# FordyceLab/magnify

Hardware: AMD Instinct MI355X
Metric: megapixels/sec through flatfield+segment+ROI-reduce; markers/sec (higher is better)
Workload: dtype u16

## Files before the change

### include/magnify_hip.h

```cpp
#ifndef MAGNIFY_HIP_H
#define MAGNIFY_HIP_H

#include <stddef.h>
#include <stdint.h>

#ifdef __cplusplus
extern "C" {
#endif

#define MG_OK 0
#define MG_EINVAL (-1)
#define MG_ELAUNCH (-2)
#define MG_EIO (-3)

#define MG_U8 0
#define MG_U16 1
#define MG_F32 2
#define MG_F64 3

#define MG_NO_EDGE 100.0f
#define MG_SCORE_SKIPPED (-2.0f)


int mg_version(void);
// ... 32 lines not shown
                                    double dark, const void* d_dark, int dark_dtype,
                                    double flat, const void* d_flat, int flat_dtype,
                                    const double* d_max2, void* d_image, double* d_minmax, void* stream);

int mg_flatfield_apply_stitch_shift(const void* d_tiles, int dtype, int64_t n_planes, int n_tile_rows, int n_tile_cols,
                                    int ty, int tx, int overlap, int apply_flatfield, int planes_per_group,
                                    double dark, const void* d_dark, int dark_dtype,
                                    double flat, const void* d_flat, int flat_dtype,
                                    const double* d_max2, void* d_image, double* d_minmax,
                                    const int32_t* d_shift, int n_tables, int n_time, int blend, void* stream);


int64_t mg_seam_sums_scratch_bytes(int64_t n_planes, int n_tile_rows, int n_tile_cols, int ty, int tx, int overlap,
                                   int max_shift);
int mg_seam_sums(const void* d_planes, int dtype, int64_t n_planes, int n_tile_rows, int n_tile_cols, int ty, int tx,
                 int overlap, int max_shift, void* d_sums, void* d_fixed, void* d_scratch, int64_t scratch_bytes,
                 void* stream);


int mg_track_beads(const void* d_planes, int dtype, int n_t, int64_t plane_stride, int h, int w, int t_ref,
                   const int32_t* d_beads, int m, int half, int max_drift, int32_t* d_shift, double* d_score,
                   void* d_sums, void* d_fixed, void* stream);

int mg_track_beads_based(const void* d_planes, int dtype, int n_t, int64_t plane_stride, int h, int w, int t_ref,
                         const int32_t* d_beads, int m, int half, int max_drift, const int32_t* d_base,
                         int32_t* d_shift, double* d_score, void* d_sums, void* d_fixed, void* stream);

int mg_bin_planes(const void* d_planes, int dtype, int n_t, int64_t plane_stride, int h, int w, int bin,
                  float* d_out, void* stream);

int mg_plane_minmax(const void* d_src, int dtype, int n_planes, int64_t plane_stride, int h, int w,
                    int64_t row_stride, double* d_minmax, void* stream);


int mg_affine_bilinear(const void* d_src, void* d_dst, int dtype, int64_t n_planes, int h, int w,
                       const double* matrix, const double* offset, double* d_minmax, void* stream);

int64_t mg_shading_workspace_bytes(int n, int w);
int64_t mg_shading_offset(int n, int w, int field);
int mg_shading_downsample(const void* d_tiles, int dtype, int64_t n, int ty, int tx, int w, float* d_out, void* stream);
int mg_shading_prepare(void* d_ws, int n, int w, void* stream);
int mg_shading_dct2(void* d_ws, int n, int w, const double* d_in, double* d_out, int inverse, void* stream);
int mg_shading_alm_begin(void* d_ws, int n, int w, int get_darkfield, int max_iterations, double mu, double lam_f,
                         double lam_d, double tol, double norm_f, double b_up, void* stream);
int mg_shading_alm_iterate(void* d_ws, int n, int w, int k, int get_darkfield, void* stream);
int mg_shading_reweight(void* d_ws, int n, int w, double epsilon, void* stream);
int mg_shading_upsample(const double* d_flat_w, const double* d_dark_w, int w, int ty, int tx, double* d_partial,
                        float* d_flat, float* d_dark, void* stream);
int mg_shading_apply_stitch(const void* d_tiles, int dtype, int n_fields, int64_t planes_per_field, int n_tile_rows,
                            int n_tile_cols, int ty, int tx, int overlap, const float* d_flat, const float* d_dark,
                            void* d_image, double* d_minmax, void* stream);
int mg_shading_apply_stitch_blend(const void* d_tiles, int dtype, int n_fields, int64_t planes_per_field,
                                  int n_tile_rows, int n_tile_cols, int ty, int tx, int overlap, const float* d_flat,
                                  const float* d_dark, void* d_image, double* d_minmax, void* stream);

int mg_shading_apply_stitch_shift(const void* d_tiles, int dtype, int n_fields, int64_t planes_per_field,
                                  int n_tile_rows, int n_tile_cols, int ty, int tx, int overlap, const float* d_flat,
                                  const float* d_dark, void* d_image, double* d_minmax, const int32_t* d_shift,
                                  int n_tables, int n_time, int blend, void* stream);


int mg_to_uint8_blur(const void* d_src, int dtype, int n_planes, int64_t plane_stride, int h, int w,
                     int64_t row_stride, const double* d_minmax, uint8_t* d_blur, uint8_t* d_u8, void* stream);

int mg_scharr_hist(const uint8_t* d_blur, int n_planes, int h, int w, int mode, const uint32_t* d_base,
                   uint32_t* d_hist, uint32_t* d_scratch, int64_t scratch_words, void* stream);
int64_t mg_scharr_hist_scratch_words(int n_planes, int h, int w, int mode);

int mg_to_uint8_blur_hist(const void* d_src, int dtype, int n_planes, int64_t plane_stride, int h, int w,
                          int64_t row_stride, const double* d_minmax, uint8_t* d_blur, uint8_t* d_u8, uint32_t* d_hist,
                          uint32_t* d_scratch, int64_t scratch_words, void* stream);
int64_t mg_blur_hist_scratch_words(int n_planes, int h, int w);

int mg_edge_thresholds(const uint32_t* d_hist, int n_planes, const int64_t* ranks4, float gamma_low, float gamma_high,
                       int32_t* d_thresh, float* d_quantiles, int32_t* d_unresolved, int32_t* d_state,
                       uint32_t* d_win_base, void* stream);
int mg_edge_thresholds_window(const uint32_t* d_hist_win, int n_planes, int pass, float gamma_low, float gamma_high,
                              int32_t* d_state, uint32_t* d_win_base, int32_t* d_thresh, float* d_quantiles,
                              int32_t* d_unresolved, void* stream);


int mg_canny_nms(const uint8_t* d_blur, int n_planes, int h, int w, const int32_t* d_thresh, uint32_t* d_weak,
                 uint32_t* d_strong, uint32_t* d_class, int64_t words_per_plane, void* stream);

int mg_canny_hysteresis(const uint32_t* d_weak, uint32_t* d_strong, int64_t words_per_plane, int n_planes, int h,
                        int w, uint32_t* d_changed, const uint8_t* d_flags_in, uint8_t* d_flags_out, void* stream);
int mg_hysteresis_tiles(int h, int w, int* tiles_x, int* tiles_y);

int mg_unpack_bits(const uint32_t* d_bits, int64_t words_per_plane, int n_planes, int64_t n_bits, uint8_t* d_out,
                   void* stream);

int64_t mg_edge_grid_scan_words(int n_planes, int h, int w, int grid);
int mg_edge_grid(const uint32_t* d_edge_bits, int64_t words_per_plane, int n_planes, int h, int w, int grid,
                 int32_t* d_cell_counts, int32_t* d_cell_starts, int32_t* d_num_edges, int32_t* d_coords,
                 int64_t coord_cap, uint64_t* d_scan_state, int32_t* d_edge_totals, int phases, void* stream);

int mg_edge_angles(const uint8_t* d_blur, int n_planes, int h, int w, const int32_t* d_coords, int64_t coord_cap,
                   const int32_t* d_num_edges, float* d_angle, void* stream);


int mg_dedup_layout(int h, int w, int min_r, int max_r, int* n_tile_rows, int* n_tile_cols, int64_t* n_layers,
                    int64_t* bitmap_words);

int mg_candidate_circles(const int32_t* d_coords, int64_t coord_cap, const int32_t* d_cell_starts,
                         const int32_t* d_cell_counts, const int32_t* d_num_edges, int n_planes, int h, int w,
                         int grid, const uint64_t* d_seeds, int64_t num_iter, int min_r, int max_r,
                         uint32_t* d_bitmap, int64_t bitmap_words, float* d_raw, void* stream);

int mg_candidate_keys(const int32_t* d_coords, int64_t coord_cap, const int32_t* d_cell_starts,
                      const int32_t* d_cell_counts, const int32_t* d_num_edges, int n_planes, int h, int w, int grid,
                      const uint64_t* d_seeds, int64_t num_iter, int min_r, int max_r, uint32_t* d_keys, float* d_raw,
                      void* stream);

int mg_keys_to_circles(const uint32_t* d_keys, int64_t num_iter, const int32_t* d_cell_starts,
                       const int32_t* d_cell_counts, const int32_t* d_num_edges, int n_planes, int h, int w, int grid,
                       int min_r, int max_r, uint32_t* d_unique_keys, int64_t circle_cap, int32_t* d_tile_ranges,
                       int32_t* d_num_circles, int32_t* d_layer_starts, int counters_clear, void* stream);

int mg_bitmap_to_circles(uint32_t* d_bitmap, int64_t bitmap_words, int n_planes, int h, int w, int min_r,
                         int max_r, int32_t* d_layer_offsets, int32_t* d_circles, int64_t circle_cap,
                         int32_t* d_num_circles, void* stream);

int mg_score_circles(const float* d_angle, const uint32_t* d_edge_bits, const uint32_t* d_class_bits,
                     int64_t words_per_plane, int n_planes, int h, int w, int32_t* d_circles, int64_t circle_cap,
                     const int32_t* d_layer_offsets, const uint32_t* d_unique_keys, const int32_t* d_tile_ranges,
                     int min_r, int max_r, const int32_t* d_per_rc, const double* d_per_expected,
                     const int32_t* d_per_starts, int per_total, float min_roundness, int write_skipped,
                     int dedup_centres, float* d_scores, int32_t* d_alive, int32_t* d_num_alive, int32_t* d_max_rc,
                     int32_t* d_num_scored, void* stream);

int mg_score_keyed_supported(int min_r, int max_r);
int mg_score_pair_table(uint64_t* out_entries, int cap);
int mg_score_pairs(int r, int32_t* out_rc, int cap);
int mg_score_walk_reads(int r);
int mg_score_circles_keyed(const uint8_t* d_blur, const float* d_angle, const uint32_t* d_edge_bits,
                           const uint32_t* d_class_bits, int64_t words_per_plane, int n_planes, int h, int w,
                           int32_t* d_circles, int64_t circle_cap, const uint32_t* d_unique_keys,
                           const int32_t* d_layer_starts, int min_r, int max_r, const int32_t* d_per_rc,
                           const double* d_per_expected, const int32_t* d_per_starts, int per_total,
                           const uint64_t* d_pair_table, float min_roundness, int write_skipped, float* d_scores,
                           int32_t* d_alive, int32_t* d_num_alive, int32_t* d_max_rc, int32_t* d_num_scored,
                           int32_t* d_surv_list, int64_t surv_cap, int32_t* d_num_surv, int counters_clear,
                           void* stream);

int mg_nms_rounds(const int32_t* d_circles, int64_t circle_cap, const float* d_scores, const int32_t* d_alive,
                  const int32_t* d_num_alive, const int32_t* d_max_rc, int n_planes, int min_dist,
                  const int32_t* d_ring_rc, int ring_len, uint64_t* d_grid, int64_t grid_cap, uint8_t* d_state,
                  int32_t* d_undecided, int64_t undecided_stride, int n_rounds, int counters_clear,
                  const uint32_t* d_tie_keys, int64_t max_alive, const int32_t* d_skip, void* stream);

int mg_nms_same_centre(const int32_t* d_circles, int64_t circle_cap, const float* d_scores, const int32_t* d_alive,
                       const int32_t* d_num_alive, const int32_t* d_max_rc, int n_planes, int min_dist, uint64_t* d_grid,
                       int64_t grid_cap, uint8_t* d_state, const uint32_t* d_tie_keys, int64_t max_alive,
                       const int32_t* d_skip, void* stream);

int mg_nms_cleanup(const int32_t* d_circles, int64_t circle_cap, const float* d_scores, const int32_t* d_alive,
                   const int32_t* d_num_alive, const int32_t* d_max_rc, int n_planes, int min_dist,
                   const int32_t* d_ring_rc, int ring_len, uint64_t* d_grid, int64_t grid_cap, uint8_t* d_state,
                   int64_t max_alive, const int32_t* d_skip, void* stream);

int mg_nms_sparse(const int32_t* d_circles, int64_t circle_cap, const float* d_scores, const int32_t* d_alive,
                  const int32_t* d_num_alive, const int32_t* d_max_rc, int n_planes, int min_dist, const uint32_t* d_dbits,
                  uint8_t* d_state, const uint32_t* d_tie_keys, int32_t* d_done, void* stream);
int mg_nms_sparse_max_dist(void);

int mg_collect_circles(const int32_t* d_circles, int64_t circle_cap, const float* d_scores, const int32_t* d_alive,
// ... 137 lines not shown
```

### magnify_amd/csrc/mg_edges.hip

```cpp
#include <math.h>
#include <stdlib.h>

#include <algorithm>

#include "mg_common.h"

namespace {

constexpr int TW = 256;
constexpr int TH = 64;
constexpr int NT = 256;
constexpr int RPW = 16;
constexpr int LPAD = 16;
constexpr int LS = TW + 2 * LPAD;
constexpr int CHUNKS = LS / 16;

struct U8Scale {
  double mn, top, scale, offset;
  int passthrough;
};

__device__ __forceinline__ U8Scale make_scale(const double* d_minmax, int plane) {
  U8Scale s;
  s.passthrough = (d_minmax == nullptr);
// ... 74 lines not shown
        uint8_t v[16];
        decode_chunk<T>(raw[it], sc, v);
        store_chunk(tile, j, k, v);
      }
    }
    return;
  }
  const bool rows_ok = ((row_stride * sizeof(T)) & 15) == 0;
  uint4 raw[ITER][NLD];
  bool fast[ITER];
#pragma unroll
  for (int it = 0; it < ITER; ++it) {
    const int i = threadIdx.x + it * NT;
    fast[it] = false;
    if (i < TOTAL) {
      const auto [j, k] = row_col(i, CHUNKS);
      const int gy = mg_reflect101(ty0 - HALO + j, h), gx0 = tx0 - LPAD + 16 * k;
      const T* p = base + (int64_t)gy * row_stride + gx0;
      fast[it] = rows_ok && gx0 >= 0 && gx0 + 16 <= w && (reinterpret_cast<uintptr_t>(p) & 15) == 0;
      if (fast[it]) {
#pragma unroll
        for (int q = 0; q < NLD; ++q) raw[it][q] = reinterpret_cast<const uint4*>(p)[q];
      }
    }
  }
#pragma unroll
  for (int it = 0; it < ITER; ++it) {
    const int i = threadIdx.x + it * NT;
    if (i < TOTAL) {
      const auto [j, k] = row_col(i, CHUNKS);
      uint8_t v[16];
      if (fast[it]) {
        decode_chunk<T>(raw[it], sc, v);
      } else {
        const int gy = mg_reflect101(ty0 - HALO + j, h), gx0 = tx0 - LPAD + 16 * k;
        const T* rowp = base + (int64_t)gy * row_stride;
#pragma unroll
        for (int m = 0; m < 16; ++m) {
          const int c = 16 * k + m;
          const bool needed = c >= LPAD - HALO && c < LPAD + TW + HALO;
          v[m] = needed ? to_u8<T>(rowp[mg_reflect101(gx0 + m, w)], sc) : (uint8_t)0;
        }
      }
      store_chunk(tile, j, k, v);
    }
  }
}

struct Row12 {
  uint32_t d0, d1, d2;
  __device__ __forceinline__ int at(int off) const {
    const int b = off + 4;
    const uint32_t d = b < 4 ? d0 : (b < 8 ? d1 : d2);
    return (int)((d >> (8 * (b & 3))) & 0xFFu);
  }
};
__device__ __forceinline__ Row12 read_row(const uint8_t (*tile)[LS], int r, int c0) {
  const uint32_t* p = reinterpret_cast<const uint32_t*>(&tile[r][LPAD + c0 - 4]);
  return Row12{p[0], p[1], p[2]};
}

typedef short s2 __attribute__((ext_vector_type(2)));
typedef unsigned short u2 __attribute__((ext_vector_type(2)));

__device__ __forceinline__ u2 pair_01(uint32_t d) { return __builtin_bit_cast(u2, __builtin_amdgcn_perm(0u, d, 0x0C010C00u)); }
__device__ __forceinline__ u2 pair_12(uint32_t d) { return __builtin_bit_cast(u2, __builtin_amdgcn_perm(0u, d, 0x0C020C01u)); }
__device__ __forceinline__ u2 pair_23(uint32_t d) { return __builtin_bit_cast(u2, __builtin_amdgcn_perm(0u, d, 0x0C030C02u)); }
__device__ __forceinline__ u2 pair_across(uint32_t lo, uint32_t hi) {
  return __builtin_bit_cast(u2, __builtin_amdgcn_perm(hi, lo, 0x0C040C03u));
}
__device__ __forceinline__ uint32_t pack_bytes(uint32_t p01, uint32_t p23) { return __builtin_amdgcn_perm(p23, p01, 0x06040200u); }
__device__ __forceinline__ uint32_t zip_lo(s2 x, s2 y) {
  return __builtin_amdgcn_perm(__builtin_bit_cast(uint32_t, y), __builtin_bit_cast(uint32_t, x), 0x05040100u);
}
__device__ __forceinline__ uint32_t zip_hi(s2 x, s2 y) {
  return __builtin_amdgcn_perm(__builtin_bit_cast(uint32_t, y), __builtin_bit_cast(uint32_t, x), 0x07060302u);
}

__device__ __forceinline__ uint32_t wave_from_left(uint32_t v) {
  return (uint32_t)__builtin_amdgcn_update_dpp(0, (int)v, 0x138, 0xF, 0xF, false);
}
__device__ __forceinline__ uint32_t wave_from_right(uint32_t v) {
  return (uint32_t)__builtin_amdgcn_update_dpp(0, (int)v, 0x130, 0xF, 0xF, false);
}

template <int NP>
__device__ __forceinline__ void scharr_pairs(const u2 (&a)[NP], const u2 (&b)[NP], const u2 (&c)[NP],
                                             uint32_t (&xy)[2 * (NP - 1)]) {
  s2 S[NP], D[NP];
#pragma unroll
  for (int k = 0; k < NP; ++k) {
    S[k] = __builtin_bit_cast(s2, (u2)((a[k] + c[k]) * (unsigned short)3 + b[k] * (unsigned short)10));
    D[k] = __builtin_bit_cast(s2, c[k]) - __builtin_bit_cast(s2, a[k]);
  }
#pragma unroll
  for (int jp = 0; jp < NP - 1; ++jp) {
    const s2 dxp = S[jp + 1] - S[jp];
    const s2 mid = __builtin_bit_cast(s2, __builtin_amdgcn_alignbit(__builtin_bit_cast(uint32_t, D[jp + 1]),
                                                                     __builtin_bit_cast(uint32_t, D[jp]), 16));
    const s2 dyp = (D[jp] + D[jp + 1]) * (short)3 + mid * (short)10;
    xy[2 * jp] = zip_lo(dxp, dyp);
    xy[2 * jp + 1] = zip_hi(dxp, dyp);
  }
}
__device__ __forceinline__ int grad_sq(uint32_t xy) {
  return __builtin_amdgcn_sdot2(__builtin_bit_cast(s2, xy), __builtin_bit_cast(s2, xy), 0, false);
}

template <typename T>
__global__ __launch_bounds__(NT) void k_u8_blur(const T* __restrict__ src, int64_t plane_stride, int h, int w,
                                                int64_t row_stride, const double* __restrict__ d_minmax,
                                                uint8_t* __restrict__ d_blur, uint8_t* __restrict__ d_u8) {
  __shared__ __attribute__((aligned(16))) uint8_t tile[TH + 4][LS];
  const int plane = blockIdx.z;
  const int tx0 = blockIdx.x * TW, ty0 = blockIdx.y * TH;
  const U8Scale sc = make_scale(d_minmax, plane);
  load_tile<T, 2>(src + (int64_t)plane * plane_stride, row_stride, h, w, tx0, ty0, sc, tile);
  __syncthreads();
  const int lane = threadIdx.x & 63, wave = threadIdx.x >> 6;
  const int c0 = 4 * lane, gx = tx0 + c0;
  if (gx >= w) return;
  int hs[5][4];
  uint8_t* outp = d_blur + (int64_t)plane * h * w;
  uint8_t* rawp = d_u8 ? d_u8 + (int64_t)plane * h * w : nullptr;
  const bool full = (gx + 4 <= w) && ((w & 3) == 0);
#pragma unroll
  for (int jr = 0; jr < RPW + 4; ++jr) {
    const Row12 r = read_row(tile, wave * RPW + jr, c0);
#pragma unroll
    for (int k = 0; k < 4; ++k)
#pragma unroll
      for (int q = 0; q < 4; ++q) hs[k][q] = hs[k + 1][q];
#pragma unroll
    for (int q = 0; q < 4; ++q) hs[4][q] = r.at(q - 2) + 4 * r.at(q - 1) + 6 * r.at(q) + 4 * r.at(q + 1) + r.at(q + 2);
    if (rawp && jr >= 2 && jr < RPW + 2) {
      const int gy = ty0 + wave * RPW + jr - 2;
      if (gy < h) {
        if (full) *reinterpret_cast<uint32_t*>(rawp + (int64_t)gy * w + gx) = r.d1;
        else
          for (int q = 0; q < 4 && gx + q < w; ++q) rawp[(int64_t)gy * w + gx + q] = (uint8_t)r.at(q);
      }
    }
    if (jr >= 4) {
      const int gy = ty0 + wave * RPW + jr - 4;
      if (gy < h) {
        uint32_t packed = 0;
#pragma unroll
        for (int q = 0; q < 4; ++q) {
          const int v = hs[0][q] + 4 * hs[1][q] + 6 * hs[2][q] + 4 * hs[3][q] + hs[4][q];
          packed |= (uint32_t)((v + 128) >> 8) << (8 * q);
        }
        if (full) *reinterpret_cast<uint32_t*>(outp + (int64_t)gy * w + gx) = packed;
        else
          for (int q = 0; q < 4 && gx + q < w; ++q) outp[(int64_t)gy * w + gx + q] = (uint8_t)(packed >> (8 * q));
      }
    }
  }
}

constexpr int FINE = 8192;
constexpr int COARSE = 4096;
constexpr uint32_t MG_HIST_SKIP = 0xFFFFFFFFu;

constexpr int HIST_TILES = 3;

__device__ __forceinline__ void hist_add4_pairs(const u2 (&pa)[3], const u2 (&pb2)[3], const u2 (&pc)[3], int gx, int w,
// ... 387 lines not shown
  const int plane = blockIdx.x;
  int32_t* st = d_state + (int64_t)plane * TS_WORDS;
  const int n_win = st[TS_NWIN];
  if (pass >= n_win) return;
  int32_t coarse[4], resid[4];
#pragma unroll
  for (int k = 0; k < 4; ++k) coarse[k] = st[TS_COARSE + k], resid[k] = st[TS_RESID + k];
  const int cbin = nth_window(coarse, pass);
  const uint32_t* hist = d_hist_win + (int64_t)plane * FINE;
  constexpr int PER = FINE / NT;
  uint32_t mine_v[PER];
  long long mine = 0;
#pragma unroll
  for (int j = 0; j < PER; ++j) mine_v[j] = hist[threadIdx.x * PER + j], mine += mine_v[j];
  long long run = block_exscan_i64(mine, s_pre);
  if (threadIdx.x < 4) s_pos[threadIdx.x] = 0;
  __syncthreads();
#pragma unroll
  for (int j = 0; j < PER; ++j) {
    const long long nxt = run + mine_v[j];
#pragma unroll
    for (int k = 0; k < 4; ++k)
      if (coarse[k] == cbin && run <= (long long)resid[k] && (long long)resid[k] < nxt) s_pos[k] = threadIdx.x * PER + j;
    run = nxt;
  }
  __syncthreads();
  if (threadIdx.x == 0) {
    int32_t order[4];
#pragma unroll
    for (int k = 0; k < 4; ++k) {
      order[k] = st[TS_ORDER + k];
      if (coarse[k] == cbin) order[k] = (cbin << 13) + s_pos[k], st[TS_ORDER + k] = order[k];
    }
    const int left = n_win - 1 - pass;
    d_unresolved[plane] = left | (n_win << 8);
    d_win_base[plane] = left > 0 ? (uint32_t)nth_window(coarse, pass + 1) << 13 : MG_HIST_SKIP;
    if (left == 0) finish_thresholds(order, gamma_lo, gamma_hi, plane, d_thresh, d_quantiles);
  }
}

__device__ __forceinline__ uint32_t bits_at(const uint32_t* __restrict__ bits, int64_t bit0, int n) {
  const int64_t wi = bit0 >> 5;
  const int sh = (int)(bit0 & 31);
  uint64_t two = bits[wi];
  if (sh + n > 32) two |= (uint64_t)bits[wi + 1] << 32;
  const uint32_t v = (uint32_t)(two >> sh);
  return n >= 32 ? v : (v & ((1u << n) - 1u));
}
__device__ __forceinline__ uint32_t bits_at_nb(const uint32_t* __restrict__ bits, int64_t bit0, int n) {
  const int64_t wi = bit0 >> 5;
  const int sh = (int)(bit0 & 31);
  const uint64_t two = (uint64_t)bits[wi] | ((uint64_t)bits[wi + 1] << 32);
  const uint32_t v = (uint32_t)(two >> sh);
  return n >= 32 ? v : (v & ((1u << n) - 1u));
}
__device__ __forceinline__ void bits_or(uint32_t* __restrict__ bits, int64_t bit0, uint32_t v) {
  if (!v) return;
  const int64_t wi = bit0 >> 5;
  const int sh = (int)(bit0 & 31);
  atomicOr(&bits[wi], v << sh);
  if (sh && (v >> (32 - sh))) atomicOr(&bits[wi + 1], v >> (32 - sh));
}
__device__ __forceinline__ uint32_t row_word(const uint32_t* __restrict__ bits, int h, int w, int y, int x0) {
  if (y < 0 || y >= h) return 0u;
  const int lo = max(x0, 0), hi = min(x0 + 32, w);
  if (lo >= hi) return 0u;
  return bits_at(bits, (int64_t)y * w + lo, hi - lo) << (lo - x0);
}

__device__ __forceinline__ uint32_t shl1_or(uint32_t v, uint64_t mask) {
  uint32_t out;
  uint64_t carry_out;
  asm("v_addc_co_u32_e64 %0, %1, %2, %2, %3" : "=v"(out), "=s"(carry_out) : "v"(v), "s"(mask));
  return out;
}

__device__ __forceinline__ uint32_t or_reduce8(uint32_t v) {
  v |= (uint32_t)__builtin_amdgcn_update_dpp(0, (int)v, 0xB1, 0xF, 0xF, true);
  v |= (uint32_t)__builtin_amdgcn_update_dpp(0, (int)v, 0x4E, 0xF, 0xF, true);
  v |= (uint32_t)__builtin_amdgcn_update_dpp(0, (int)v, 0x141, 0xF, 0xF, true);
  return v;
}

__global__ __launch_bounds__(NT) void k_canny_nms(const uint8_t* __restrict__ d_blur, int h, int w,
                                                  const int32_t* __restrict__ d_thresh, int64_t words_per_plane,
                                                  uint32_t* __restrict__ d_weak, uint32_t* __restrict__ d_strong,
                                                  uint32_t* __restrict__ d_class) {
  __shared__ __attribute__((aligned(16))) uint8_t tile[TH + 4][LS];
  const int plane = blockIdx.z;
  const int tx0 = blockIdx.x * TW, ty0 = blockIdx.y * TH;
  load_tile<uint8_t, 2>(d_blur + (int64_t)plane * h * w, w, h, w, tx0, ty0, make_scale(nullptr, 0), tile);
  __syncthreads();
  const int low = d_thresh[2 * plane], high = d_thresh[2 * plane + 1];
  const int lane = threadIdx.x & 63, wave = threadIdx.x >> 6;
  const int c0 = 4 * lane, gx = tx0 + c0;
  uint32_t* weak = d_weak + plane * words_per_plane;
  uint32_t* strong = d_strong + plane * words_per_plane;
  uint32_t* cls0 = d_class ? d_class + (3 * plane) * words_per_plane : nullptr;
  uint32_t* cls1 = d_class ? d_class + (3 * plane + 1) * words_per_plane : nullptr;
  uint32_t* cls2 = d_class ? d_class + (3 * plane + 2) * words_per_plane : nullptr;
  constexpr int TG22 = 13573;
  const uint32_t in_row = gx + 4 <= w ? 0xFu : ((1u << max(w - gx, 0)) - 1u);
  struct Pairs4 {
    u2 p[4];
  };
  auto unpack = [](const Row12& r) {
    Pairs4 o;
    o.p[0] = pair_23(r.d0);
    o.p[1] = pair_01(r.d1);
    o.p[2] = pair_23(r.d1);
    o.p[3] = pair_01(r.d2);
    return o;
  };
  int mg[3][6];
  uint32_t cxy[2][4];
  Pairs4 ua = unpack(read_row(tile, wave * RPW, c0)), ub = unpack(read_row(tile, wave * RPW + 1, c0));
#pragma unroll
  for (int jr = 2; jr < RPW + 4; ++jr) {
    const Pairs4 uc = unpack(read_row(tile, wave * RPW + jr, c0));
    const int ym = ty0 - 2 + wave * RPW + jr - 1;
#pragma unroll
    for (int k = 0; k < 6; ++k) mg[0][k] = mg[1][k], mg[1][k] = mg[2][k];
#pragma unroll
    for (int q = 0; q < 4; ++q) cxy[0][q] = cxy[1][q];
    {
      uint32_t xy[6];
      scharr_pairs(ua.p, ub.p, uc.p, xy);
      const bool row_in = ym >= 0 && ym < h;
#pragma unroll
      for (int k = 0; k < 6; ++k) {
        const int x = gx + k - 1;
        const int m = grad_sq(xy[k]);
        mg[2][k] = (row_in && x >= 0 && x < w) ? m : 0;
        if (k >= 1 && k <= 4) cxy[1][k - 1] = xy[k];
      }
    }
    ua = ub;
    ub = uc;
    if (jr < 4) continue;
    const int yo = ym - 1;
    uint32_t wb = 0, sb = 0, cb0 = 0, cb1 = 0, cb2 = 0;
    if (yo < h) {
#pragma unroll
      for (int q = 3; q >= 0; --q) {
        const int m = mg[1][q + 1];
        const int xs = (int)(int16_t)(cxy[0][q] & 0xFFFFu), ys = (int)cxy[0][q] >> 16;
        const int x = abs(xs), ay = abs(ys), y = ay << 15;
        const int tg22x = x * TG22;
        const int tg67x = tg22x + (x << 16);
        const uint64_t horiz = __ballot(y < tg22x);
        const uint64_t vert = __ballot(y > tg67x) & ~horiz;
        const bool neg_b = (xs ^ ys) < 0;
        const uint64_t neg = __ballot(neg_b);
        const uint64_t ok_h = __ballot(m > mg[1][q]) & __ballot(m >= mg[1][q + 2]);
        const uint64_t ok_v = __ballot(m > mg[0][q + 1]) & __ballot(m >= mg[2][q + 1]);
        const uint64_t ok_d = __ballot(m > mg[0][q]) & __ballot(m > mg[2][q + 2]);
        const uint64_t ok_n = __ballot(m > mg[0][q + 2]) & __ballot(m > mg[2][q]);
        const uint64_t is_max = (horiz & ok_h) | (vert & ok_v) | (~(horiz | vert) & ((neg & ok_n) | (~neg & ok_d)));
        const uint64_t cand = is_max & __ballot(m > low) & __ballot(gx + q < w);
        wb = shl1_or(wb, cand);
        sb = shl1_or(sb, cand & __ballot(m > high));
        const bool le_b = ay <= x, ge_b = ay >= x;
        const uint64_t le = __ballot(le_b), ge = __ballot(ge_b);
        cb0 = shl1_or(cb0, (neg & le) | (~neg & ge));
        cb1 = shl1_or(cb1, neg);
        const bool lowq = neg_b ? le_b : !ge_b;
        const int sq = lowq ? x + ay : ay - x;
        const uint64_t upper = __ballot(sq * sq > 2 * x * x);
        cb2 = shl1_or(cb2, neg ^ upper);
      }
    }
    wb = or_reduce8(wb << (4 * (lane & 7)));
    sb = or_reduce8(sb << (4 * (lane & 7)));
    if (d_class) {
      cb0 = or_reduce8((cb0 & in_row) << (4 * (lane & 7)));
      cb1 = or_reduce8((cb1 & in_row) << (4 * (lane & 7)));
      cb2 = or_reduce8((cb2 & in_row) << (4 * (lane & 7)));
    }
    if ((lane & 7) == 0 && yo < h && gx < w) {
      const int64_t bit0 = (int64_t)yo * w + gx;
      if ((bit0 & 31) == 0 && gx + 32 <= w) {
        weak[bit0 >> 5] = wb;
        strong[bit0 >> 5] = sb;
        if (d_class) {
          cls0[bit0 >> 5] = cb0;
          cls1[bit0 >> 5] = cb1;
          cls2[bit0 >> 5] = cb2;
        }
      } else {
        bits_or(weak, bit0, wb);
        bits_or(strong, bit0, sb);
        if (d_class) {
          bits_or(cls0, bit0, cb0);
          bits_or(cls1, bit0, cb1);
          bits_or(cls2, bit0, cb2);
        }
      }
    }
  }
}

constexpr int HW = TW / 32;
constexpr int HTH = 256;

__device__ __forceinline__ bool hyst_interior(int r, int k) { return r >= 1 && r <= HTH && k >= 1 && k <= HW; }
__device__ __forceinline__ uint32_t lds_interior(const uint32_t (*a)[HW + 2], int r, int k) {
  return hyst_interior(r, k) ? a[r][k] : 0u;
}
template <typename At>
__device__ __forceinline__ uint32_t dilate3x3(At at, int r, int k) {
  uint32_t dil = 0;
#pragma unroll
  for (int dr = -1; dr <= 1; ++dr) {
    const uint32_t c = at(r + dr, k), l = at(r + dr, k - 1), rt = at(r + dr, k + 1);
    dil |= c | (c << 1) | (c >> 1) | (l >> 31) | (rt << 31);
  }
  return dil;
}

__global__ __launch_bounds__(NT) void k_hysteresis(const uint32_t* __restrict__ d_weak, uint32_t* __restrict__ d_strong,
                                                   int64_t words_per_plane, int h, int w,
                                                   uint32_t* __restrict__ d_changed,
                                                   const uint8_t* __restrict__ d_flags_in,
                                                   uint8_t* __restrict__ d_flags_out) {
  __shared__ uint32_t st[HTH + 2][HW + 2];
  __shared__ uint32_t wk[HTH + 2][HW + 2];
  __shared__ uint32_t s_mark;
  const int plane = blockIdx.z;
  const int tx0 = blockIdx.x * TW, ty0 = blockIdx.y * HTH;
  const int ntx = gridDim.x, nty = gridDim.y;
  if (d_flags_in && !d_flags_in[(int64_t)plane * ntx * nty + blockIdx.y * ntx + blockIdx.x]) return;
  const uint32_t* weak = d_weak + plane * words_per_plane;
  uint32_t* strong = d_strong + plane * words_per_plane;
  int pending = 0;
  if ((w & 31) == 0) {
    constexpr int TOTAL = (HTH + 2) * (HW + 2), ITER = (TOTAL + NT - 1) / NT;
    uint32_t sv[ITER], wv[ITER];
#pragma unroll
    for (int it = 0; it < ITER; ++it) {
      const int i = min((int)threadIdx.x + it * NT, TOTAL - 1);
      const auto [r, kk] = row_col(i, HW + 2);
      const int y = ty0 - 1 + r, x = tx0 - 32 + 32 * kk;
      const bool in = y >= 0 && y < h && x >= 0 && x < w;
      const int64_t wi = in ? ((int64_t)y * w + x) >> 5 : 0;
      sv[it] = strong[wi];
      wv[it] = weak[wi];
      if (!in) sv[it] = 0u, wv[it] = 0u;
    }
#pragma unroll
    for (int it = 0; it < ITER; ++it) {
      const int i = threadIdx.x + it * NT;
      if (i < TOTAL) {
        const auto [r, kk] = row_col(i, HW + 2);
        st[r][kk] = sv[it];
        wk[r][kk] = wv[it];
        if (hyst_interior(r, kk)) pending |= (wv[it] & ~sv[it]) != 0;
      }
    }
  } else {
    for (int i = threadIdx.x; i < (HTH + 2) * (HW + 2); i += NT) {
      const auto [r, kk] = row_col(i, HW + 2);
      const uint32_t sv = row_word(strong, h, w, ty0 - 1 + r, tx0 - 32 + 32 * kk);
      const uint32_t wv = row_word(weak, h, w, ty0 - 1 + r, tx0 - 32 + 32 * kk);
      st[r][kk] = sv;
      wk[r][kk] = wv;
      if (hyst_interior(r, kk)) pending |= (wv & ~sv) != 0;
    }
  }
  if (threadIdx.x == 0) s_mark = 0u;
  if (!__syncthreads_or(pending)) return;
  constexpr int WPT = HTH * HW / NT;
  static_assert(WPT * NT == HTH * HW, "the tile's words must divide evenly over the threads");
  const int k = (threadIdx.x & (HW - 1)) + 1, r0 = WPT * (threadIdx.x / HW) + 1;
  uint32_t first[WPT];
#pragma unroll
  for (int j = 0; j < WPT; ++j) first[j] = st[r0 + j][k];
  int again;
  do {
    int changed = 0;
#pragma unroll
    for (int j = 0; j < WPT; ++j) {
      const int r = r0 + j;
// ... 326 lines not shown
      return MG_ELAUNCH;
    attr_set = true;
  }
  const int split = d_scratch ? 1 : 0;
  if (split) {
    hipLaunchKernelGGL(k_scharr_hist<true>, g, dim3(NT), (size_t)n_bins * 2, mg_stream(stream), d_blur, h, w, mode,
                       d_base, n_bins, d_hist, d_scratch, split);
    MG_CHECK_LAUNCH();
  }
  hipLaunchKernelGGL(k_scharr_hist<false>, t, dim3(NT), lds, mg_stream(stream), d_blur, h, w, mode, d_base, n_bins,
                     d_hist, d_scratch, split);
  MG_CHECK_LAUNCH();
  if (!d_scratch) return MG_OK;
  return launch_hist_reduce(d_scratch, (int)(g.x * g.y), n_bins, n_planes, d_hist, mode == 1 ? d_base : nullptr, mg_stream(stream));
}

static bool blur_hist_fused(const void* d_src, int dtype, int64_t plane_stride, int h, int w, int64_t row_stride,
                            const uint8_t* d_blur, const uint8_t* d_u8) {
  if (d_u8 || (dtype != MG_U8 && dtype != MG_U16) || h < 2 || w < 8 || (w & 3)) return false;
  const int64_t esz = dtype == MG_U8 ? 1 : 2;
  return (reinterpret_cast<uintptr_t>(d_src) % (4 * esz)) == 0 && plane_stride % 4 == 0 && row_stride % 4 == 0 &&
         (reinterpret_cast<uintptr_t>(d_blur) & 3) == 0;
}

extern "C" int64_t mg_blur_hist_scratch_words(int n_planes, int h, int w) {
  if (n_planes < 0 || h < 0 || w < 0) return -1;
  const int64_t fused = (int64_t)n_planes * ((w + FW - 1) / FW) * ((h + FH - 1) / FH) * ((FINE + COARSE) / 2);
  return std::max(fused, mg_scharr_hist_scratch_words(n_planes, h, w, 0));
}

extern "C" int mg_to_uint8_blur_hist(const void* d_src, int dtype, int n_planes, int64_t plane_stride, int h, int w,
                                     int64_t row_stride, const double* d_minmax, uint8_t* d_blur, uint8_t* d_u8,
                                     uint32_t* d_hist, uint32_t* d_scratch, int64_t scratch_words, void* stream) {
  if (!d_src || !d_blur || !d_hist || n_planes < 0 || h < 0 || w < 0) return MG_EINVAL;
  if (!d_minmax && dtype != MG_U8) return MG_EINVAL;
  if (n_planes == 0 || h == 0 || w == 0) return MG_OK;
  if (d_scratch && scratch_words < mg_blur_hist_scratch_words(n_planes, h, w)) return MG_EINVAL;
  static const bool off = getenv("MG_NO_BLUR_HIST") != nullptr;
  if (off || !d_scratch || !blur_hist_fused(d_src, dtype, plane_stride, h, w, row_stride, d_blur, d_u8)) {
    const int rc = mg_to_uint8_blur(d_src, dtype, n_planes, plane_stride, h, w, row_stride, d_minmax, d_blur, d_u8, stream);
    if (rc != MG_OK) return rc;
    return mg_scharr_hist(d_blur, n_planes, h, w, 0, nullptr, d_hist, d_scratch, scratch_words, stream);
  }
  const dim3 g((w + FW - 1) / FW, (h + FH - 1) / FH, n_planes);
  if (!grid_ok(g)) return MG_EINVAL;
  hipStream_t s = mg_stream(stream);
  constexpr int n_bins = FINE + COARSE;
  if (dtype == MG_U8)
    hipLaunchKernelGGL((k_blur_hist<uint8_t>), g, dim3(NT), (size_t)n_bins * 2, s, (const uint8_t*)d_src, plane_stride, h, w,
                       row_stride, d_minmax, d_blur, d_scratch);
  else
    hipLaunchKernelGGL((k_blur_hist<uint16_t>), g, dim3(NT), (size_t)n_bins * 2, s, (const uint16_t*)d_src, plane_stride, h,
                       w, row_stride, d_minmax, d_blur, d_scratch);
  MG_CHECK_LAUNCH();
  return launch_hist_reduce(d_scratch, (int)(g.x * g.y), n_bins, n_planes, d_hist, nullptr, s);
}

extern "C" int mg_edge_thresholds(const uint32_t* d_hist, int n_planes, const int64_t* ranks4, float gamma_low,
                                  float gamma_high, int32_t* d_thresh, float* d_quantiles, int32_t* d_unresolved,
                                  int32_t* d_state, uint32_t* d_win_base, void* stream) {
  if (!d_hist || !ranks4 || !d_thresh || !d_quantiles || !d_unresolved || n_planes < 0) return MG_EINVAL;
  if ((d_state == nullptr) != (d_win_base == nullptr)) return MG_EINVAL;
  if (n_planes == 0) return MG_OK;
  hipLaunchKernelGGL(k_edge_thresholds, dim3(n_planes), dim3(NT), 0, mg_stream(stream), d_hist, FINE, FINE + COARSE,
                     (long long)ranks4[0], (long long)ranks4[1], (long long)ranks4[2], (long long)ranks4[3], gamma_low,
                     gamma_high, d_thresh, d_quantiles, d_unresolved, d_state, d_win_base);
  MG_CHECK_LAUNCH();
  return MG_OK;
}

extern "C" int mg_edge_thresholds_window(const uint32_t* d_hist_win, int n_planes, int pass, float gamma_low,
                                         float gamma_high, int32_t* d_state, uint32_t* d_win_base, int32_t* d_thresh,
                                         float* d_quantiles, int32_t* d_unresolved, void* stream) {
  if (!d_hist_win || !d_state || !d_win_base || !d_thresh || !d_quantiles || !d_unresolved || n_planes < 0 || pass < 0 ||
      pass > 3)
    return MG_EINVAL;
  if (n_planes == 0) return MG_OK;
  hipLaunchKernelGGL(k_window_resolve, dim3(n_planes), dim3(NT), 0, mg_stream(stream), d_hist_win, pass, gamma_low,
                     gamma_high, d_state, d_win_base, d_thresh, d_quantiles, d_unresolved);
  MG_CHECK_LAUNCH();
  return MG_OK;
}

extern "C" int mg_canny_nms(const uint8_t* d_blur, int n_planes, int h, int w, const int32_t* d_thresh,
                            uint32_t* d_weak, uint32_t* d_strong, uint32_t* d_class, int64_t words_per_plane,
                            void* stream) {
  if (!d_blur || !d_thresh || !d_weak || !d_strong || n_planes < 0 || h < 0 || w < 0) return MG_EINVAL;
  if (n_planes == 0 || h == 0 || w == 0) return MG_OK;
  if (!words_ok(words_per_plane, h, w)) return MG_EINVAL;
  const dim3 g = tile_grid(h, w, n_planes);
  if (!grid_ok(g)) return MG_EINVAL;
  hipStream_t s = mg_stream(stream);
  const size_t bytes = (size_t)n_planes * words_per_plane * 4;
  if ((w & 31) && (mg_zero_async(d_weak, bytes, s) != hipSuccess || mg_zero_async(d_strong, bytes, s) != hipSuccess ||
                   (d_class && mg_zero_async(d_class, 3 * bytes, s) != hipSuccess)))
    return MG_ELAUNCH;
  hipLaunchKernelGGL(k_canny_nms, g, dim3(NT), 0, s, d_blur, h, w, d_thresh, words_per_plane, d_weak, d_strong,
                     d_class);
  MG_CHECK_LAUNCH();
  return MG_OK;
}

extern "C" int mg_canny_hysteresis(const uint32_t* d_weak, uint32_t* d_strong, int64_t words_per_plane, int n_planes,
                                   int h, int w, uint32_t* d_changed, const uint8_t* d_flags_in, uint8_t* d_flags_out,
                                   void* stream) {
  if (!d_weak || !d_strong || !d_changed || n_planes < 0 || h < 0 || w < 0) return MG_EINVAL;
  if (n_planes == 0 || h == 0 || w == 0) return MG_OK;
  if (!words_ok(words_per_plane, h, w)) return MG_EINVAL;
  const dim3 g = hysteresis_grid(h, w, n_planes);
  if (!grid_ok(g)) return MG_EINVAL;
  hipLaunchKernelGGL(k_hysteresis, g, dim3(NT), 0, mg_stream(stream), d_weak, d_strong, words_per_plane, h, w,
                     d_changed, d_flags_in, d_flags_out);
  MG_CHECK_LAUNCH();
  return MG_OK;
}

extern "C" int mg_hysteresis_tiles(int h, int w, int* tiles_x, int* tiles_y) {
  if (!tiles_x || !tiles_y) return MG_EINVAL;
  const dim3 g = hysteresis_grid(h, w, 1);
  *tiles_x = (int)g.x;
  *tiles_y = (int)g.y;
  return MG_OK;
}

extern "C" int mg_unpack_bits(const uint32_t* d_bits, int64_t words_per_plane, int n_planes, int64_t n_bits,
                              uint8_t* d_out, void* stream) {
  if (!d_bits || !d_out || n_planes < 0 || n_planes > 65535 || n_bits < 0 || words_per_plane * 32 < n_bits)
    return MG_EINVAL;
  if (n_planes == 0 || n_bits == 0) return MG_OK;
  const int bx = (int)std::min<int64_t>((n_bits + NT - 1) / NT, 4096);
  hipLaunchKernelGGL(k_unpack_bits, dim3(bx, n_planes), dim3(NT), 0, mg_stream(stream), d_bits, words_per_plane, n_bits,
                     d_out);
  MG_CHECK_LAUNCH();
  return MG_OK;
}

extern "C" int64_t mg_edge_grid_scan_words(int n_planes, int h, int w, int grid) {
  if (n_planes < 0 || h < 0 || w < 0 || grid <= 0) return -1;
  const int64_t n_cells = (int64_t)((h + grid - 1) / grid) * ((w + grid - 1) / grid);
  return (int64_t)n_planes * ((n_cells + SCAN_CHUNK - 1) / SCAN_CHUNK + 1);
}

extern "C" int mg_edge_grid(const uint32_t* d_edge_bits, int64_t words_per_plane, int n_planes, int h, int w, int grid,
                            int32_t* d_cell_counts, int32_t* d_cell_starts, int32_t* d_num_edges, int32_t* d_coords,
                            int64_t coord_cap, uint64_t* d_scan_state, int32_t* d_edge_totals, int phases, void* stream) {
  if (!d_edge_bits || !d_cell_counts || !d_cell_starts || !d_num_edges || n_planes < 0 || grid <= 0 || coord_cap < 0 ||
      n_planes > 65535 || phases < 1 || phases > 3 || ((phases & 2) && !d_coords))
    return MG_EINVAL;
  if (n_planes == 0) return MG_OK;
  if (!words_ok(words_per_plane, h, w)) return MG_EINVAL;
  const int gr = (h + grid - 1) / grid, gc = (w + grid - 1) / grid, n_cells = gr * gc;
  hipStream_t s = mg_stream(stream);
  if (phases & 1) {
    const int n_chunks = (n_cells + SCAN_CHUNK - 1) / SCAN_CHUNK;
    const bool chunked = d_scan_state && n_chunks > 1 && n_chunks <= 65535 && n_chunks + 1 <= n_cells;
    if (n_cells > 0) {
      hipLaunchKernelGGL(k_cell_count, dim3((n_cells + NT - 1) / NT, n_planes), dim3(NT), 0, s, d_edge_bits,
                         words_per_plane, h, w, grid, gc, n_cells, d_cell_counts,
                         chunked ? reinterpret_cast<unsigned long long*>(d_scan_state) : nullptr, n_chunks + 1);
      MG_CHECK_LAUNCH();
    }
    const int64_t limit = (phases & 2) ? coord_cap : -1;
    if (chunked) {
      hipLaunchKernelGGL(k_cell_scan_chunks, dim3(n_chunks, n_planes), dim3(1024), 0, s, d_cell_counts, n_cells,
                         d_cell_starts, d_num_edges, d_edge_totals, limit, reinterpret_cast<unsigned long long*>(d_scan_state));
    } else {
      hipLaunchKernelGGL(k_cell_scan, dim3(n_planes), dim3(1024), 0, s, d_cell_counts, n_cells, d_cell_starts, d_num_edges,
                         d_edge_totals, limit);
    }
    MG_CHECK_LAUNCH();
  }
  if ((phases & 2) && n_cells > 0) {
    if (grid <= 64) {
      const int64_t groups = (n_cells + 64 / grid - 1) / (64 / grid);
      const int64_t waves = (groups + FILL_TRIPS - 1) / FILL_TRIPS;
      hipLaunchKernelGGL(k_cell_fill_rows, dim3((unsigned)((waves + NT / 64 - 1) / (NT / 64)), n_planes), dim3(NT), 0, s,
                         d_edge_bits, words_per_plane, h, w, grid, gc, n_cells, d_cell_starts, d_coords, coord_cap);
    } else {
      hipLaunchKernelGGL(k_cell_fill, dim3((n_cells + NT - 1) / NT, n_planes), dim3(NT), 0, s, d_edge_bits,
                         words_per_plane, h, w, grid, gc, n_cells, d_cell_starts, d_coords, coord_cap);
    }
    MG_CHECK_LAUNCH();
// ... 16 lines not shown
```

Measured before the change: 225,600.

## Add LDS-free strip-based Canny NMS kernel with register row streaming

Adds a new NMS path where each wave processes a 256-wide, 64-row strip. Rows are loaded straight from global memory into registers, prefetched four rows ahead, and halo columns are exchanged with DPP lane shifts instead of an LDS tile and barrier. Interior strips use vectorized 32-bit loads in a separate launch, and edge strips use reflected byte loads. The NMS math is factored into a helper that reuses neighbour comparison ballots across rows to save ballot work. The cost is two launches, more register pressure, and recomputing gradients on overlapping halo rows.

Measured after the change: 229,300, median of 6. 1.6% higher.

```diff
diff --git a/include/magnify_hip.h b/include/magnify_hip.h
--- a/include/magnify_hip.h
+++ b/include/magnify_hip.h
@@ -138,6 +138,7 @@
 
 int mg_canny_nms(const uint8_t* d_blur, int n_planes, int h, int w, const int32_t* d_thresh, uint32_t* d_weak,
                  uint32_t* d_strong, uint32_t* d_class, int64_t words_per_plane, void* stream);
+int mg_canny_nms_strips(int w, int* strip_w, int* wave_rows, int* group_rows);
 
 int mg_canny_hysteresis(const uint32_t* d_weak, uint32_t* d_strong, int64_t words_per_plane, int n_planes, int h,
                         int w, uint32_t* d_changed, const uint8_t* d_flags_in, uint8_t* d_flags_out, void* stream);
diff --git a/magnify_amd/csrc/mg_edges.hip b/magnify_amd/csrc/mg_edges.hip
--- a/magnify_amd/csrc/mg_edges.hip
+++ b/magnify_amd/csrc/mg_edges.hip
@@ -180,6 +180,13 @@
 }
 __device__ __forceinline__ uint32_t wave_from_right(uint32_t v) {
   return (uint32_t)__builtin_amdgcn_update_dpp(0, (int)v, 0x130, 0xF, 0xF, false);
+}
+
+__device__ __forceinline__ uint32_t wave_from_left(uint32_t v, uint32_t fill) {
+  return (uint32_t)__builtin_amdgcn_update_dpp((int)fill, (int)v, 0x138, 0xF, 0xF, false);
+}
+__device__ __forceinline__ uint32_t wave_from_right(uint32_t v, uint32_t fill) {
+  return (uint32_t)__builtin_amdgcn_update_dpp((int)fill, (int)v, 0x130, 0xF, 0xF, false);
 }
 
 template <int NP>
@@ -733,6 +740,55 @@
   return v;
 }
 
+struct NmsBits {
+  uint32_t wb, sb, cb0, cb1, cb2;
+};
+__device__ __forceinline__ void nms_rising(const int (&above)[6], const int (&row)[6], uint64_t (&up)[4]) {
+#pragma unroll
+  for (int q = 0; q < 4; ++q) up[q] = __ballot(row[q + 1] > above[q + 1]);
+}
+__device__ __forceinline__ NmsBits nms_row(const int (&mg)[3][6], const uint32_t (&xy)[4], int low, int high,
+                                           const uint64_t (&inside)[4], uint64_t (&up)[4]) {
+  constexpr int TG22 = 13573;
+  NmsBits o{0u, 0u, 0u, 0u, 0u};
+  uint64_t gt[5], dn[4];
+#pragma unroll
+  for (int k = 0; k < 5; ++k) gt[k] = __ballot(mg[1][k + 1] > mg[1][k]);
+#pragma unroll
+  for (int q = 0; q < 4; ++q) dn[q] = __ballot(mg[2][q + 1] > mg[1][q + 1]);
+#pragma unroll
+  for (int q = 3; q >= 0; --q) {
+    const int m = mg[1][q + 1];
+    const s2 g = __builtin_bit_cast(s2, xy[q]);
+    const uint32_t au = __builtin_bit_cast(uint32_t, __builtin_elementwise_max(g, (s2)(0) - g));
+    const int x = (int)(au & 0xFFFFu), ay = (int)(au >> 16);
+    const int y = ay << 15, tg22x = __mul24(x, TG22), tg67x = tg22x + (int)(au << 16);
+    const uint64_t horiz = __ballot(y < tg22x);
+    const uint64_t vert = __ballot(y > tg67x) & ~horiz;
+    const uint64_t neg = __ballot((int16_t)(xy[q] & 0xFFFFu) < 0) ^ __ballot((int)xy[q] < 0);
+    const uint64_t ok_h = gt[q] & ~gt[q + 1];
+    const uint64_t ok_v = up[q] & ~dn[q];
+    const uint64_t ok_d = __ballot(m > mg[0][q]) & __ballot(m > mg[2][q + 2]);
+    const uint64_t ok_n = __ballot(m > mg[0][q + 2]) & __ballot(m > mg[2][q]);
+    const uint64_t is_max = (horiz & ok_h) | (vert & ok_v) | (~(horiz | vert) & ((neg & ok_n) | (~neg & ok_d)));
+    const uint64_t cand = is_max & __ballot(m > low) & inside[q];
+    o.wb = shl1_or(o.wb, cand);
+    o.sb = shl1_or(o.sb, cand & __ballot(m > high));
+    const int dif = x - ay, sum = x + ay;
+    const uint64_t le = __ballot(dif >= 0), ge = __ballot(dif <= 0);
+    o.cb0 = shl1_or(o.cb0, (neg & le) | (~neg & ge));
+    o.cb1 = shl1_or(o.cb1, neg);
+    const int xx2 = 2 * __mul24(x, x);
+    const uint64_t lowq = (neg & le) | ~(neg | ge);
+    const uint64_t upper = (lowq & __ballot(__mul24(sum, sum) > xx2)) |
+                           (~lowq & __ballot(__mul24(dif, dif) > xx2));
+    o.cb2 = shl1_or(o.cb2, neg ^ upper);
+  }
+#pragma unroll
+  for (int q = 0; q < 4; ++q) up[q] = dn[q];
+  return o;
+}
+
 __global__ __launch_bounds__(NT) void k_canny_nms(const uint8_t* __restrict__ d_blur, int h, int w,
                                                   const int32_t* __restrict__ d_thresh, int64_t words_per_plane,
                                                   uint32_t* __restrict__ d_weak, uint32_t* __restrict__ d_strong,
@@ -743,15 +799,18 @@
   load_tile<uint8_t, 2>(d_blur + (int64_t)plane * h * w, w, h, w, tx0, ty0, make_scale(nullptr, 0), tile);
   __syncthreads();
   const int low = d_thresh[2 * plane], high = d_thresh[2 * plane + 1];
-  const int lane = threadIdx.x & 63, wave = threadIdx.x >> 6;
+  const int lane = threadIdx.x & 63;
+  const int wave = __builtin_amdgcn_readfirstlane(threadIdx.x >> 6);
   const int c0 = 4 * lane, gx = tx0 + c0;
   uint32_t* weak = d_weak + plane * words_per_plane;
   uint32_t* strong = d_strong + plane * words_per_plane;
   uint32_t* cls0 = d_class ? d_class + (3 * plane) * words_per_plane : nullptr;
   uint32_t* cls1 = d_class ? d_class + (3 * plane + 1) * words_per_plane : nullptr;
   uint32_t* cls2 = d_class ? d_class + (3 * plane + 2) * words_per_plane : nullptr;
-  constexpr int TG22 = 13573;
   const uint32_t in_row = gx + 4 <= w ? 0xFu : ((1u << max(w - gx, 0)) - 1u);
+  uint64_t inside[4], up[4];
+#pragma unroll
+  for (int q = 0; q < 4; ++q) inside[q] = __ballot(gx + q < w), up[q] = 0;
   struct Pairs4 {
     u2 p[4];
   };
@@ -788,38 +847,13 @@
     }
     ua = ub;
     ub = uc;
+    if (jr == 3) nms_rising(mg[1], mg[2], up);
     if (jr < 4) continue;
     const int yo = ym - 1;
     uint32_t wb = 0, sb = 0, cb0 = 0, cb1 = 0, cb2 = 0;
     if (yo < h) {
-#pragma unroll
-      for (int q = 3; q >= 0; --q) {
-        const int m = mg[1][q + 1];
-        const int xs = (int)(int16_t)(cxy[0][q] & 0xFFFFu), ys = (int)cxy[0][q] >> 16;
-        const int x = abs(xs), ay = abs(ys), y = ay << 15;
-        const int tg22x = x * TG22;
-        const int tg67x = tg22x + (x << 16);
-        const uint64_t horiz = __ballot(y < tg22x);
-        const uint64_t vert = __ballot(y > tg67x) & ~horiz;
-        const bool neg_b = (xs ^ ys) < 0;
-        const uint64_t neg = __ballot(neg_b);
-        const uint64_t ok_h = __ballot(m > mg[1][q]) & __ballot(m >= mg[1][q + 2]);
-        const uint64_t ok_v = __ballot(m > mg[0][q + 1]) & __ballot(m >= mg[2][q + 1]);
-        const uint64_t ok_d = __ballot(m > mg[0][q]) & __ballot(m > mg[2][q + 2]);
-        const uint64_t ok_n = __ballot(m > mg[0][q + 2]) & __ballot(m > mg[2][q]);
-        const uint64_t is_max = (horiz & ok_h) | (vert & ok_v) | (~(horiz | vert) & ((neg & ok_n) | (~neg & ok_d)));
-        const uint64_t cand = is_max & __ballot(m > low) & __ballot(gx + q < w);
-        wb = shl1_or(wb, cand);
-        sb = shl1_or(sb, cand & __ballot(m > high));
-        const bool le_b = ay <= x, ge_b = ay >= x;
-        const uint64_t le = __ballot(le_b), ge = __ballot(ge_b);
-        cb0 = shl1_or(cb0, (neg & le) | (~neg & ge));
-        cb1 = shl1_or(cb1, neg);
-        const bool lowq = neg_b ? le_b : !ge_b;
-        const int sq = lowq ? x + ay : ay - x;
-        const uint64_t upper = __ballot(sq * sq > 2 * x * x);
-        cb2 = shl1_or(cb2, neg ^ upper);
-      }
+      const NmsBits o = nms_row(mg, cxy[0], low, high, inside, up);
+      wb = o.wb, sb = o.sb, cb0 = o.cb0, cb1 = o.cb1, cb2 = o.cb2;
     }
     wb = or_reduce8(wb << (4 * (lane & 7)));
     sb = or_reduce8(sb << (4 * (lane & 7)));
@@ -849,6 +883,159 @@
       }
     }
   }
+}
+
+constexpr int NW = 256;
+constexpr int NR = 64;
+constexpr int NH = (NT / 64) * NR;
+constexpr int NB = 4;
+static_assert((NR + 4) % NB == 0 && NB >= 4, "row loop");
+
+template <bool VEC>
+__device__ __forceinline__ void nms_strip(const uint8_t* __restrict__ pb, int h, int w, int y0, int tx0, int low, int high,
+                                          uint32_t* __restrict__ weak, uint32_t* __restrict__ strong,
+                                          uint32_t* __restrict__ cls0, uint32_t* __restrict__ cls1,
+                                          uint32_t* __restrict__ cls2) {
+  const int lane = threadIdx.x & 63;
+  const int cx = tx0 + 4 * lane;
+  const bool left_half = lane < 32;
+  const int ex = left_half ? tx0 - 4 : tx0 + NW;
+  uint32_t col[4], ecol[4];
+#pragma unroll
+  for (int q = 0; q < 4; ++q) {
+    col[q] = VEC ? (uint32_t)(cx + q) : (uint32_t)mg_reflect101(cx + q, w);
+    ecol[q] = VEC ? (uint32_t)(ex + q) : (uint32_t)mg_reflect101(ex + q, w);
+  }
+  const int n_out = min(NR, h - y0), n_rows = n_out + 4;
+  struct Row {
+    uint32_t d, e;
+  };
+  auto load = [&](int j) {
+    int ry = y0 - 2 + j;
+    ry = ry < 0 ? -ry : ry;
+    ry = ry >= h ? 2 * h - 2 - ry : ry;
+    ry = min(max(ry, 0), h - 1);
+    const uint8_t* rowp = pb + (int64_t)ry * w;
+    Row r;
+    if (VEC) {
+      r.d = *reinterpret_cast<const uint32_t*>(rowp + col[0]);
+      r.e = *reinterpret_cast<const uint32_t*>(rowp + ecol[0]);
+    } else {
+      r.d = (uint32_t)rowp[col[0]] | ((uint32_t)rowp[col[1]] << 8) | ((uint32_t)rowp[col[2]] << 16) | ((uint32_t)rowp[col[3]] << 24);
+      r.e = (uint32_t)rowp[ecol[0]] | ((uint32_t)rowp[ecol[1]] << 8) | ((uint32_t)rowp[ecol[2]] << 16) | ((uint32_t)rowp[ecol[3]] << 24);
+    }
+    return r;
+  };
+  const uint32_t sel_a = left_half ? 0x0C070C06u : 0x0C040C03u, sel_b = left_half ? 0x0C010C00u : 0x0C060C05u;
+  const bool in_img = cx < w;
+  const bool edge_in = left_half ? tx0 > 0 : tx0 + NW < w;
+  uint64_t inside[4], up[4];
+#pragma unroll
+  for (int q = 0; q < 4; ++q) inside[q] = __ballot(in_img), up[q] = 0;
+  u2 P[3][3];
+  u2 Q[3][2];
+  int mg[3][6];
+  uint32_t cxy[2][4];
+#pragma unroll
+  for (int k = 0; k < 3; ++k) {
+    P[k][0] = P[k][1] = P[k][2] = Q[k][0] = Q[k][1] = (u2)(0);
+#pragma unroll
+    for (int c = 0; c < 6; ++c) mg[k][c] = 0;
+  }
+#pragma unroll
+  for (int q = 0; q < 4; ++q) cxy[0][q] = cxy[1][q] = 0u;
+  Row cur[NB], nxt[NB];
+#pragma unroll
+  for (int b = 0; b < NB; ++b) cur[b] = load(min(b, n_rows - 1));
+#pragma unroll 1
+  for (int j0 = 0; j0 < n_rows; j0 += NB) {
+#pragma unroll
+    for (int b = 0; b < NB; ++b) nxt[b] = load(min(j0 + NB + b, n_rows - 1));
+#pragma unroll
+    for (int b = 0; b < NB; ++b) {
+      const int j = j0 + b;
+      const uint32_t d1 = cur[b].d, e = cur[b].e;
+      const uint32_t d0 = wave_from_left(d1, e), d2 = wave_from_right(d1, e);
+#pragma unroll
+      for (int k = 0; k < 2; ++k) {
+        P[k][0] = P[k + 1][0], P[k][1] = P[k + 1][1], P[k][2] = P[k + 1][2];
+        Q[k][0] = Q[k + 1][0], Q[k][1] = Q[k + 1][1];
+      }
+      P[2][0] = pair_across(d0, d1);
+      P[2][1] = pair_12(d1);
+      P[2][2] = pair_across(d1, d2);
+      Q[2][0] = __builtin_bit_cast(u2, __builtin_amdgcn_perm(e, d1, sel_a));
+      Q[2][1] = __builtin_bit_cast(u2, __builtin_amdgcn_perm(e, d1, sel_b));
+      const int ym = y0 - 3 + j;
+      const bool row_in = ym >= 0 && ym < h;
+#pragma unroll
+      for (int c = 0; c < 6; ++c) mg[0][c] = mg[1][c], mg[1][c] = mg[2][c];
+#pragma unroll
+      for (int q = 0; q < 4; ++q) cxy[0][q] = cxy[1][q];
+      uint32_t exy[2];
+      scharr_pairs(P[0], P[1], P[2], cxy[1]);
+      scharr_pairs(Q[0], Q[1], Q[2], exy);
+#pragma unroll
+      for (int q = 0; q < 4; ++q) mg[2][q + 1] = (row_in && in_img) ? grad_sq(cxy[1][q]) : 0;
+      const uint32_t em = (row_in && edge_in) ? (uint32_t)grad_sq(exy[0]) : 0u;
+      mg[2][0] = (int)wave_from_left((uint32_t)mg[2][4], em);
+      mg[2][5] = (int)wave_from_right((uint32_t)mg[2][1], em);
+      if (j == 3) nms_rising(mg[1], mg[2], up);
+      if (j0 == 0 || j >= n_rows) continue;
+      const int yo = y0 - 4 + j;
+      const NmsBits o = nms_row(mg, cxy[0], low, high, inside, up);
+      const uint32_t keep = in_img ? 0xFu : 0u;
+      const uint32_t wb = or_reduce8(o.wb << (4 * (lane & 7))), sb = or_reduce8(o.sb << (4 * (lane & 7)));
+      uint32_t cb0 = 0, cb1 = 0, cb2 = 0;
+      if (cls0) {
+        cb0 = or_reduce8((o.cb0 & keep) << (4 * (lane & 7)));
+        cb1 = or_reduce8((o.cb1 & keep) << (4 * (lane & 7)));
+        cb2 = or_reduce8((o.cb2 & keep) << (4 * (lane & 7)));
+      }
+      if ((lane & 7) == 0 && in_img) {
+        const int64_t bit0 = (int64_t)yo * w + cx;
+        if ((bit0 & 31) == 0 && cx + 32 <= w) {
+          weak[bit0 >> 5] = wb;
+          strong[bit0 >> 5] = sb;
+          if (cls0) {
+            cls0[bit0 >> 5] = cb0;
+            cls1[bit0 >> 5] = cb1;
+            cls2[bit0 >> 5] = cb2;
+          }
+        } else {
+          bits_or(weak, bit0, wb);
+          bits_or(strong, bit0, sb);
+          if (cls0) {
+            bits_or(cls0, bit0, cb0);
+            bits_or(cls1, bit0, cb1);
+            bits_or(cls2, bit0, cb2);
+          }
+        }
+      }
+    }
+#pragma unroll
+    for (int b = 0; b < NB; ++b) cur[b] = nxt[b];
+  }
+}
+
+template <bool VEC>
+__global__ __launch_bounds__(NT) __attribute__((amdgpu_waves_per_eu(VEC ? 5 : 4)))
+void k_canny_nms_strips(const uint8_t* __restrict__ d_blur, int h, int w, int x_first, int x_jump,
+                        const int32_t* __restrict__ d_thresh, int64_t words_per_plane, uint32_t* __restrict__ d_weak,
+                        uint32_t* __restrict__ d_strong, uint32_t* __restrict__ d_class) {
+  const int plane = blockIdx.z;
+  const int tx0 = ((int)blockIdx.x + x_first + (blockIdx.x ? x_jump : 0)) * NW;
+  const int wave = __builtin_amdgcn_readfirstlane(threadIdx.x >> 6);
+  const int y0 = blockIdx.y * NH + wave * NR;
+  if (y0 >= h) return;
+  const int low = d_thresh[2 * plane], high = d_thresh[2 * plane + 1];
+  const uint8_t* pb = d_blur + (int64_t)plane * h * w;
+  uint32_t* weak = d_weak + plane * words_per_plane;
+  uint32_t* strong = d_strong + plane * words_per_plane;
+  uint32_t* cls0 = d_class ? d_class + (3 * plane) * words_per_plane : nullptr;
+  uint32_t* cls1 = d_class ? d_class + (3 * plane + 1) * words_per_plane : nullptr;
+  uint32_t* cls2 = d_class ? d_class + (3 * plane + 2) * words_per_plane : nullptr;
+  nms_strip<VEC>(pb, h, w, y0, tx0, low, high, weak, strong, cls0, cls1, cls2);
 }
 
 constexpr int HW = TW / 32;
@@ -1341,22 +1528,44 @@
   return MG_OK;
 }
 
+static bool nms_strips(const uint8_t* d_blur, int w) { return (w & 3) == 0 && (reinterpret_cast<uintptr_t>(d_blur) & 3) == 0; }
+
 extern "C" int mg_canny_nms(const uint8_t* d_blur, int n_planes, int h, int w, const int32_t* d_thresh,
                             uint32_t* d_weak, uint32_t* d_strong, uint32_t* d_class, int64_t words_per_plane,
                             void* stream) {
   if (!d_blur || !d_thresh || !d_weak || !d_strong || n_planes < 0 || h < 0 || w < 0) return MG_EINVAL;
   if (n_planes == 0 || h == 0 || w == 0) return MG_OK;
   if (!words_ok(words_per_plane, h, w)) return MG_EINVAL;
-  const dim3 g = tile_grid(h, w, n_planes);
+  const bool strips = nms_strips(d_blur, w);
+  const int n_strips = (w + NW - 1) / NW, n_vec = std::max(0, (w - NW - 4) / NW);
+  const dim3 g = strips ? dim3(n_strips - n_vec, (h + NH - 1) / NH, n_planes) : tile_grid(h, w, n_planes);
   if (!grid_ok(g)) return MG_EINVAL;
   hipStream_t s = mg_stream(stream);
   const size_t bytes = (size_t)n_planes * words_per_plane * 4;
   if ((w & 31) && (mg_zero_async(d_weak, bytes, s) != hipSuccess || mg_zero_async(d_strong, bytes, s) != hipSuccess ||
                    (d_class && mg_zero_async(d_class, 3 * bytes, s) != hipSuccess)))
     return MG_ELAUNCH;
-  hipLaunchKernelGGL(k_canny_nms, g, dim3(NT), 0, s, d_blur, h, w, d_thresh, words_per_plane, d_weak, d_strong,
-                     d_class);
+  if (strips) {
+    if (n_vec > 0) {
+      hipLaunchKernelGGL(k_canny_nms_strips<true>, dim3(n_vec, g.y, g.z), dim3(NT), 0, s, d_blur, h, w, 1, 0, d_thresh,
+                         words_per_plane, d_weak, d_strong, d_class);
+      MG_CHECK_LAUNCH();
+    }
+    hipLaunchKernelGGL(k_canny_nms_strips<false>, g, dim3(NT), 0, s, d_blur, h, w, 0, n_vec, d_thresh, words_per_plane,
+                       d_weak, d_strong, d_class);
+  } else
+    hipLaunchKernelGGL(k_canny_nms, g, dim3(NT), 0, s, d_blur, h, w, d_thresh, words_per_plane, d_weak, d_strong,
+                       d_class);
   MG_CHECK_LAUNCH();
+  return MG_OK;
+}
+
+extern "C" int mg_canny_nms_strips(int w, int* strip_w, int* wave_rows, int* group_rows) {
+  if (!strip_w || !wave_rows || !group_rows || w < 0) return MG_EINVAL;
+  const bool strips = nms_strips(nullptr, w);
+  *strip_w = strips ? NW : TW;
+  *wave_rows = strips ? NR : RPW;
+  *group_rows = strips ? NH : TH;
   return MG_OK;
 }
 
```
